# rogosprojects/klogs

Measured on AMD Instinct MI355X. Metric: filtered log GB/s (whole node) at 1/2/4/8 MI355X; % of HBM peak, higher is better.
Workload: dtype u8

## Files before the change

klogs_amd/csrc/klf_kernels.hip:

```cpp
#include <hip/hip_ext.h>
#include <hip/hip_runtime.h>

#include <cstdio>
#include <cstdlib>
#include <cstring>
#include <type_traits>

#include "klf_kernels.hpp"
#include "klf_ts.hpp"

namespace klf {
namespace {

#ifndef KLF_TIMELINE
#define KLF_TIMELINE 0
#endif
__device__ uint32_t g_abl_waves;
#if KLF_TIMELINE
__device__ uint64_t g_timeline[300000 * 8];
__device__ uint32_t g_lb_rounds, g_lb_spins;
#define KLF_STAMP(tile, k) do { if (threadIdx.x == 0 && (tile) < 300000) g_timeline[(size_t)(tile) * 8 + (k)] = __builtin_amdgcn_s_memtime(); } while (0)
#else
#define KLF_STAMP(tile, k) do { } while (0)
#endif
// ... 165 lines not shown
  }
  return x;
}

__device__ __forceinline__ uint32_t xad(uint32_t x, uint32_t c, uint32_t d) {
  uint32_t r;
  asm("v_xad_u32 %0, %1, %2, %3" : "=v"(r) : "v"(x), "s"(c), "v"(d));
  return r;
}
__device__ __forceinline__ uint32_t any_eq16(const uint4& v, uint32_t c4) {
  const uint32_t m = 0xFEFEFEFFu;
  return (xad(v.x, c4, m) | xad(v.y, c4, m) | xad(v.z, c4, m) | xad(v.w, c4, m)) & 0x80808080u;
}
__device__ __forceinline__ uint32_t eq_mask16(const uint4& v, uint32_t c4) {
  auto z = [c4](uint32_t x) {
    const uint32_t y = x ^ c4;
    const uint32_t f = ~(((y & 0x7F7F7F7Fu) + 0x7F7F7F7Fu) | y) & 0x80808080u;
    return (f * 0x00204081u) >> 28;
  };
  return z(v.x) | (z(v.y) << 4) | (z(v.z) << 8) | (z(v.w) << 12);
}

__device__ __forceinline__ uint32_t nor_and(uint32_t a, uint32_t b, uint32_t c) {
  uint32_t r;
  asm("v_bitop3_b32 %0, %1, %2, %3 bitop3:0x02" : "=v"(r) : "v"(a), "v"(b), "s"(c));
  return r;
}
__device__ __forceinline__ uint32_t eq_mask16_nl(const uint4& v) {
  auto z = [](uint32_t x) {
    const uint32_t t = xad(x & 0x7F7F7F7Fu, 0x0A0A0A0Au, 0x7F7F7F7Fu);
    const uint32_t f = nor_and(t, x, 0x80808080u);
    return (f * 0x00204081u) >> 28;
  };
  return z(v.x) | (z(v.y) << 4) | (z(v.z) << 8) | (z(v.w) << 12);
}

template <class T>
__device__ __forceinline__ T wave_max(T x) {
#pragma unroll
  for (int d = 32; d >= 1; d >>= 1) {
    const T o = __shfl_xor(x, d, 64);
    x = o > x ? o : x;
  }
  return x;
}

__device__ __forceinline__ void wave_lds_sync() { asm volatile("s_waitcnt lgkmcnt(0)" ::: "memory"); }

__global__ __launch_bounds__(256) void k_tiles(const SegDesc* segs, uint32_t nsegs, uint32_t ntiles,
                                               uint32_t* tile_seg) {
  for (uint32_t tile = blockIdx.x * 256 + threadIdx.x; tile < ntiles; tile += gridDim.x * 256)
    tile_seg[tile] = find_seg_by_tile(segs, nsegs, tile);
}

__device__ __forceinline__ uint32_t mul_hi_u24(uint32_t a, uint32_t b) {
  uint32_t r;
  asm("v_mul_hi_u32_u24 %0, %1, %2" : "=v"(r) : "s"(b), "v"(a));
  return r;
}
__device__ __forceinline__ uint32_t mul_u24(uint32_t a, uint32_t b) {
  uint32_t r;
  asm("v_mul_u32_u24 %0, %1, %2" : "=v"(r) : "s"(b), "v"(a));
  return r;
}
__device__ __forceinline__ uint32_t mad_u24(uint32_t a, uint32_t b, uint32_t c) {
  uint32_t r;
  asm("v_mad_u32_u24 %0, %1, %2, %3" : "=v"(r) : "v"(a), "s"(b), "v"(c));
  return r;
}
__device__ __forceinline__ uint32_t bfe_u32(uint32_t a, uint32_t off, uint32_t width) {
  uint32_t r;
  asm("v_bfe_u32 %0, %1, %2, %3" : "=v"(r) : "v"(a), "n"(off), "n"(width));
  return r;
}
__device__ __forceinline__ uint32_t shr_byte1(uint32_t w, uint32_t h) {
  uint32_t r;
  asm("v_lshrrev_b32_sdwa %0, %1, %2 dst_sel:DWORD dst_unused:UNUSED_PAD src0_sel:BYTE_1 src1_sel:DWORD"
      : "=v"(r) : "v"(h), "v"(w));
  return r;
}
#ifndef KLF_PARSE_UNALIGNED
#define KLF_PARSE_UNALIGNED 1
#endif
__device__ __forceinline__ bool parse_fast(const uint8_t* lds, uint32_t o, const uint32_t (&cut)[6], bool& since_ok) {
  uint32_t w[8];
  if (KLF_PARSE_UNALIGNED) {
    typedef uint32_t u32x4 __attribute__((ext_vector_type(4)));
    u32x4 x0, x1;
    __builtin_memcpy(&x0, lds + o, 16);
    __builtin_memcpy(&x1, lds + o + 16, 16);
    w[0] = x0.x; w[1] = x0.y; w[2] = x0.z; w[3] = x0.w;
    w[4] = x1.x; w[5] = x1.y; w[6] = x1.z; w[7] = x1.w;
  } else {
    const uint32_t* s32 = reinterpret_cast<const uint32_t*>(lds);
    const uint32_t base = o >> 2, sh = o & 3u;
    uint32_t prev = s32[base];
#pragma unroll
    for (int j = 0; j < 8; ++j) {
      const uint32_t nx = s32[base + j + 1];
      w[j] = __builtin_amdgcn_alignbyte(nx, prev, sh);
      prev = nx;
    }
  }
  const uint32_t sep = ((w[1] ^ 0x2D00002Du) & 0xFF0000FFu) | ((w[2] ^ 0x00540000u) & 0x00FF0000u) |
                       ((w[3] ^ 0x00003A00u) & 0x0000FF00u) | ((w[4] ^ 0x2E00003Au) & 0xFF0000FFu) |
                       ((w[7] ^ 0x00205A00u) & 0x00FFFF00u);
  const uint32_t p0 = __builtin_amdgcn_perm(0u, w[0], 0x00010203u);
  const uint32_t p1 = __builtin_amdgcn_perm(w[2], w[1], 0x01020405u);
  const uint32_t p2 = __builtin_amdgcn_perm(w[3], w[2], 0x03040607u);
  const uint32_t p3 = __builtin_amdgcn_perm(w[5], w[4], 0x01020405u);
  const uint32_t p4 = __builtin_amdgcn_perm(w[6], w[5], 0x02030405u);
  const uint32_t p5 = __builtin_amdgcn_perm(w[7], w[6], 0x02030C04u) | 0x00003000u;
  const uint32_t hi = ((p0 ^ 0x30303030u) | (p1 ^ 0x30303030u) | (p2 ^ 0x30303030u) | (p3 ^ 0x30303030u) |
                       (p4 ^ 0x30303030u) | (p5 ^ 0x30303030u)) & 0xF0F0F0F0u;
  const uint32_t lo = ((p0 + 0x06060606u) | (p1 + 0x06060606u) | (p2 + 0x06060606u) | (p3 + 0x06060606u) |
                       (p4 + 0x06060606u) | (p5 + 0x06060606u)) & 0x40404040u;
  if ((sep | hi | lo) != 0u) return false;
  if (p0 - 0x31393730u > 0x32303939u - 0x31393730u) return false;
  if ((p1 >> 16) - 0x3031u > 0x3132u - 0x3031u) return false;
  if ((p2 >> 16) > 0x3233u || (p2 & 0xFFFFu) > 0x3539u || (p3 >> 16) > 0x3539u) return false;
  if ((p1 & 0xFFFFu) - 0x3031u > 0x3238u - 0x3031u) {
    const uint32_t day = ((p1 >> 8) & 15u) * 10u + (p1 & 15u);
    const uint32_t month = ((p1 >> 24) & 15u) * 10u + ((p1 >> 16) & 15u);
    const uint32_t yy = ((p0 >> 8) & 15u) * 10u + (p0 & 15u);
    const uint32_t dim = month == 2u ? 28u + ((yy & 3u) == 0u ? 1u : 0u) : 30u + ((month + (month >> 3)) & 1u);
    if (day - 1u >= dim) return false;
  }
  const uint64_t a0 = (uint64_t)p0 << 32 | p1, a1 = (uint64_t)p2 << 32 | p3, a2 = (uint64_t)p4 << 32 | p5;
  const uint64_t c0 = (uint64_t)cut[0] << 32 | cut[1], c1 = (uint64_t)cut[2] << 32 | cut[3],
                 c2 = (uint64_t)cut[4] << 32 | cut[5];
  since_ok = a0 > c0 || (a0 == c0 && (a1 > c1 || (a1 == c1 && a2 >= c2)));
  return true;
}

#ifndef KLF_ABL
#define KLF_ABL 0
#endif
#ifndef KLF_SCAN_NT
#define KLF_SCAN_NT 1
#endif
#ifndef KLF_SCAN_PRIO
#define KLF_SCAN_PRIO 0
#endif
#ifndef KLF_NL_MASK
#define KLF_NL_MASK 1
#endif
#ifndef KLF_SCAN_BALLOT
#define KLF_SCAN_BALLOT 1
#endif
#ifndef KLF_SCAN_PACKSUM
#define KLF_SCAN_PACKSUM 1
#endif
#ifndef KLF_VERIFY_PAR
#define KLF_VERIFY_PAR 0
#endif
#ifndef KLF_HIT_INLINE
#define KLF_HIT_INLINE 0
#endif
#ifndef KLF_TS_INLINE
#define KLF_TS_INLINE 1
#endif
#ifndef KLF_SCAN_SUMSKIP
#define KLF_SCAN_SUMSKIP 1
#endif
typedef uint32_t klf_v4u __attribute__((ext_vector_type(4)));
__device__ __forceinline__ uint4 ld_nt(const uint4* p) {
  const klf_v4u v = __builtin_nontemporal_load(reinterpret_cast<const klf_v4u*>(p));
  return make_uint4(v.x, v.y, v.z, v.w);
}
#ifndef KLF_CG_NT
#define KLF_CG_NT 0
#endif
#ifndef KLF_CG_GRID
#define KLF_CG_GRID 8
#endif
#ifndef KLF_CG_PF2
#define KLF_CG_PF2 1
#endif
#ifndef KLF_COPY_U
#define KLF_COPY_U 1
#endif
#ifndef KLF_ANY_BATCH
#define KLF_ANY_BATCH 8
#endif
#ifndef KLF_SCAN_OCC
#define KLF_SCAN_OCC 3
#endif
constexpr int kScanPlain = 0, kScanLit = 1, kScanGen = 2;

__device__ __forceinline__ void copy_tile_runs(const uint8_t* s_buf, uint32_t* s_run, uint16_t* s_map, uint32_t nr,
                                               uint32_t kept, uint64_t obase, uint8_t* out, int lane);

template <int MODE, int QS, int QK, int QQ = 4, bool QA = false, bool FUSE = false>
__global__ __launch_bounds__(kThreads, MODE == kScanGen ? 3 : KLF_SCAN_OCC) void k_scan(RunArgs a, const uint32_t* __restrict__ tseg,
                                                               const SegDesc* __restrict__ segs) {
  static_assert(!FUSE || MODE == kScanPlain, "the fused compaction runs in the plain scan");
  constexpr bool LIT = MODE == kScanLit;
  constexpr bool GEN = MODE == kScanGen;
  constexpr bool ANC = GEN && QA;
  static_assert(QQ == 3 || QQ == 4, "3- or 4-byte grams");
  constexpr int kWaves = kThreads / 64;
  constexpr int kRows = kTile / 1024;
  constexpr int kPad = FUSE ? 16 : 0;
  __shared__ __attribute__((aligned(16))) uint8_t s_tile_all[kWaves][kPad + kTile + kHalo];
  __shared__ __attribute__((aligned(16))) uint32_t s_frun_all[FUSE ? kWaves : 1][FUSE ? kTcRuns : 1];
  __shared__ __attribute__((aligned(16))) uint16_t s_fmap_all[FUSE ? kWaves : 1][FUSE ? kTcChunks : 8];
  __shared__ __attribute__((aligned(16))) uint32_t s_list_all[kWaves][kSlotStride];
  __shared__ __attribute__((aligned(16))) uint32_t s_lit[kMaxFusedLiteral / 4 + 1];
  __shared__ uint4 s_gstat[GEN ? 1 : kWaves][kScanGroup];
  __shared__ uint32_t s_qf[GEN ? kQfWords : 1];
  __shared__ uint32_t s_h2[GEN ? kWaves : 1][1];
  const int t = threadIdx.x, lane = t & 63, wv = __builtin_amdgcn_readfirstlane(t >> 6);
  uint8_t* s_tile = s_tile_all[wv] + kPad;
  uint32_t* s_list = s_list_all[wv];
  uint32_t* err_flag = a.counters + 2;
  for (uint32_t i = t; i < kMaxFusedLiteral / 4 + 1; i += kThreads)
    s_lit[i] = (LIT && i < (a.lit_len + 3) / 4) ? a.lit_words[i] : 0u;
  if (GEN)
    for (uint32_t i = t; i < kQfWords; i += kThreads) s_qf[i] = a.pats.qf_bitmap[i];
  __syncthreads();
  const uint32_t nwaves = gridDim.x * kWaves;
  const bool abl = (KLF_ABL != 0) &&
                   __hip_atomic_load(&g_abl_waves, __ATOMIC_RELAXED, __HIP_MEMORY_SCOPE_AGENT) >= nwaves;
#define ABL(x) ((KLF_ABL & (x)) && abl)

  static_assert(kRows == 8, "KLF_ROWS lists the 8 prefetch rows");
#define KLF_ROWS(X) X(0) X(1) X(2) X(3) X(4) X(5) X(6) X(7)
#define KLF_DECL(r) uint4 pf##r;
  KLF_ROWS(KLF_DECL)
#undef KLF_DECL
#define KLF_LOAD(r) pf##r = (KLF_SCAN_NT && MODE != kScanPlain) ? ld_nt(&gp[r * 64 + lane]) : gp[r * 64 + lane];
#define KLF_STORE(r) l[r * 64 + lane] = pf##r;
  uint4 pfh = make_uint4(0, 0, 0, 0);
  auto next_tile = [&](uint32_t x) -> uint32_t {
    return (FUSE || (x % kScanGroup) != kScanGroup - 1) ? x + 1 : x + 1 + kScanGroup * (nwaves - 1);
  };
  const uint32_t gw = blockIdx.x * kWaves + wv;
  uint32_t tile = FUSE ? gw * a.fuse_range : gw * kScanGroup;
  const uint32_t tile_end = FUSE ? (tile + a.fuse_range < a.ntiles ? tile + a.fuse_range : a.ntiles) : a.ntiles;
  const uint32_t range_t0 = tile;
  uint4 stv = make_uint4(0, 0, 0, 0);
  uint32_t pf_s = 0;
  SegDesc pf_sd{};
  if (tile < a.ntiles) {
    pf_s = tseg[tile];
    pf_sd = segs[pf_s];
    const uint4* gp = reinterpret_cast<const uint4*>(a.bytes + pf_sd.base + (uint64_t)(tile - pf_sd.tile0) * kTile);
    KLF_ROWS(KLF_LOAD)
    if (lane < kHalo / 16) pfh = (KLF_SCAN_NT && MODE != kScanPlain) ? ld_nt(&gp[kTile / 16 + lane]) : gp[kTile / 16 + lane];
  }
  {
    const __amdgpu_buffer_rsrc_t none = __builtin_amdgcn_make_buffer_rsrc(a.slots, 0, 0, 0x00020000);
    __builtin_amdgcn_raw_buffer_store_b32(0u, none, 0x7FFF0000u, 0, 0);
  }
  bool any_defer = false;
  uint32_t wp_cur = 0, wp_end = 0;
  bool fz_known = false, fz_sel = false, fz_res_set = false;
  int32_t fz_crel = -1;
  uint64_t fz_obase = 0, fz_estart = 0, fz_res = 0, fz_part = 0, fz_rbase = 0;
  uint32_t fz_ext = 0;
  if (FUSE && tile < tile_end) {
    fz_rbase = pf_sd.base + (uint64_t)(tile - pf_sd.tile0) * kTile;
    fz_ext = a.fuse_ext0[gw];
  }
  auto fz_close = [&]() __attribute__((always_inline)) {
    if (!fz_res_set) {
      fz_res = fz_part;
      fz_res_set = true;
      fz_estart = fz_obase = fz_rbase + fz_part;
    }
    if (lane == 0) {
      a.fuse_ext[2 * (size_t)fz_ext] = fz_estart;
      a.fuse_ext[2 * (size_t)fz_ext + 1] = fz_obase - fz_estart;
    }
  };
  for (; tile < tile_end; tile = next_tile(tile)) {
    const uint32_t s = pf_s;
    const SegDesc sd = pf_sd;
    const int64_t rel_lo = (int64_t)(tile - sd.tile0) * kTile;
    const int64_t seg_len = (int64_t)sd.len;
    const int32_t tile_len = (int32_t)(seg_len - rel_lo < kTile ? seg_len - rel_lo : kTile);
    const bool first = rel_lo == 0;
    const bool last = rel_lo + kTile >= seg_len;
    const uint8_t* segp = a.bytes + sd.base;

    if (KLF_SCAN_PRIO) __builtin_amdgcn_s_setprio(KLF_SCAN_PRIO);
    {
      uint4* l = reinterpret_cast<uint4*>(s_tile);
      KLF_ROWS(KLF_STORE)
      if (lane < kHalo / 16) l[kTile / 16 + lane] = pfh;
      const uint32_t nx = next_tile(tile);
      if (nx < tile_end) {
        if (nx - sd.tile0 >= sd.ntiles) {
          pf_s = tseg[nx];
          pf_sd = segs[pf_s];
        }
        const uint4* gp = reinterpret_cast<const uint4*>(a.bytes + pf_sd.base + (uint64_t)(nx - pf_sd.tile0) * kTile);
        KLF_ROWS(KLF_LOAD)
        if (lane < kHalo / 16) pfh = (KLF_SCAN_NT && MODE != kScanPlain) ? ld_nt(&gp[kTile / 16 + lane]) : gp[kTile / 16 + lane];
      }
    }
    if (KLF_SCAN_PRIO) __builtin_amdgcn_s_setprio(0);
    wave_lds_sync();

    const uint32_t my0 = (uint32_t)lane * kLaneBytes;
    const int nvalid_s = tile_len - (int)my0;
    const int nvalid = nvalid_s <= 0 ? 0 : (nvalid_s >= kLaneBytes ? kLaneBytes : nvalid_s);
    const uint32_t pat = ANC ? a.pats.qf_anc_byte : a.lit_anchor_byte * 0x01010101u;
    const uint32_t afold = ANC ? a.pats.qf_anc_fold : 0u;
    auto or4 = [](const uint4& x, uint32_t f) { return make_uint4(x.x | f, x.y | f, x.z | f, x.w | f); };
    uint32_t nlc = 0, anc = 0;
    {
      const uint32_t rot = ((uint32_t)lane >> 1) & 7u;
#pragma unroll
      for (int v0 = 0; v0 < 8; v0 += KLF_ANY_BATCH) {
        uint4 xs[KLF_ANY_BATCH];
#pragma unroll
        for (int v = 0; v < KLF_ANY_BATCH; ++v)
          xs[v] = *reinterpret_cast<const uint4*>(s_tile + my0 + 16u * (((uint32_t)(v0 + v) + rot) & 7u));
#pragma unroll
        for (int v = 0; v < KLF_ANY_BATCH; ++v) {
          const uint32_t c = ((uint32_t)(v0 + v) + rot) & 7u;
          nlc |= any_eq16(xs[v], 0x0A0A0A0Au) ? (1u << c) : 0u;
          if (LIT && !ABL(2)) anc |= any_eq16(xs[v], pat) ? (1u << c) : 0u;
          if (ANC) anc |= any_eq16(afold ? or4(xs[v], afold) : xs[v], pat) ? (1u << c) : 0u;
        }
      }
      if (nvalid < kLaneBytes) {
        const uint32_t vm = (1u << ((nvalid + 15) >> 4)) - 1u;
        nlc &= vm;
        anc &= vm;
      }
    }
    if (ABL(64)) {
      asm volatile("" ::"v"(nlc | anc) : "memory");
      continue;
    }
    auto clip = [&](uint32_t e, uint32_t c) -> uint32_t {
      const int nv = nvalid - 16 * (int)c;
      return nv >= 16 ? e : (nv <= 0 ? 0u : (e & ((1u << nv) - 1u)));
    };
    uint32_t em[4] = {0u, 0u, 0u, 0u};
    for (uint32_t m = nlc; m; m &= m - 1u) {
      const uint32_t c = (uint32_t)__builtin_ctz(m);
      const uint4 x = *reinterpret_cast<const uint4*>(s_tile + my0 + 16u * c);
      const uint32_t e = clip(KLF_NL_MASK ? eq_mask16_nl(x) : eq_mask16(x, 0x0A0A0A0Au), c) << ((c & 1u) * 16u);
      const uint32_t q = c >> 1;
      em[0] |= q == 0 ? e : 0u;
      em[1] |= q == 1 ? e : 0u;
      em[2] |= q == 2 ? e : 0u;
      em[3] |= q == 3 ? e : 0u;
    }
    uint32_t st[4] = {em[0], em[1], em[2], em[3]};
    if (last && nvalid > 0 && (int)my0 + nvalid == tile_len) {
      const uint32_t eb = (uint32_t)nvalid - 1u, q = eb >> 5, bit = 1u << (eb & 31u);
      bool nl_at_end = false;
#pragma unroll
      for (int k = 0; k < 4; ++k)
        if ((uint32_t)k == q) {
          nl_at_end = (em[k] & bit) != 0u;
          em[k] |= bit;
          st[k] &= ~bit;
        }
      if (!abl) a.segout[s].frag = nl_at_end ? 0 : 1;
    }
    const uint32_t cnt = (uint32_t)(__popc(em[0]) + __popc(em[1]) + __popc(em[2]) + __popc(em[3]));
    const uint32_t incl = (KLF_SCAN_BALLOT && !__any(cnt > 1u))
                              ? cnt + __builtin_amdgcn_mbcnt_hi((uint32_t)(__ballot(cnt != 0u) >> 32),
                                                                __builtin_amdgcn_mbcnt_lo((uint32_t)__ballot(cnt != 0u), 0u))
                              : wave_incl_scan_add(cnt, lane);
    const uint32_t agg = (uint32_t)__builtin_amdgcn_readlane((int)incl, 63);
    const uint32_t k0 = first ? 0 : 1;
    const uint32_t k1 = last ? agg : agg + 1;
    const uint32_t nlines = k1 > k0 ? k1 - k0 : 0;
    const bool dense = nlines > (uint32_t)kSlots;
    uint32_t pool_base = 0;
    if (dense) {
      uint32_t pb = 0;
      if (lane == 0 && !abl) {
        pb = atomicAdd(&a.counters[kCtrPool], (nlines + 31u) & ~31u);
        if ((uint64_t)pb + nlines > a.pool_cap) atomicOr(err_flag, 1u);
      }
      pool_base = (uint32_t)__builtin_amdgcn_readlane((int)pb, 0);
    }
    const bool pool_ok = !dense || (uint64_t)pool_base + nlines <= a.pool_cap;
    uint32_t* const trec = a.slots + (size_t)tile * kRecStride;
    uint32_t* gslot = dense ? a.pool + pool_base : trec + kRecHead;

    uint32_t n_parsed = 0, n_since = 0, n_defer = 0, carry = 0, n_hit = 0;
    auto work = [&](uint32_t* list) __attribute__((always_inline)) {
      if (first && lane == 0) list[0] = 0u;
      {
        uint32_t kk = incl - cnt;
#pragma unroll
        for (int q = 0; q < 4; ++q) {
          for (uint32_t ev = em[q]; ev; ev &= ev - 1u) {
            const uint32_t b = (uint32_t)__builtin_ctz(ev);
            ++kk;
            if ((st[q] >> b) & 1u) list[kk - k0] = my0 + 32u * q + b + 1u;
          }
        }
      }
      if (dense) __threadfence_block();
      wave_lds_sync();
      for (uint32_t b0 = 0; b0 < nlines; b0 += 64) {
        const uint32_t j = b0 + (uint32_t)lane;
        if (j < nlines) {
          const uint32_t off = list[j];
          bool so = false, fast = false;
          if (ABL(1)) {
            fast = so = true;
          } else if (rel_lo + (int64_t)off + 31 <= seg_len) {
            fast = parse_fast(s_tile, off, a.since_dig, so);
          }
          if (FUSE && !fast) {
            TsResult tr;
            uint32_t plen = 0;
            const bool ok = parse_line_prefix(GlobalBytes{segp, rel_lo + (int64_t)off, seg_len}, tr, plen);
            const bool so2 = ok && !time_before(tr.sec, tr.nsec, a.since_sec, a.since_nsec);
            list[j] = off | ((uint32_t)make_meta(ok, so2, ok ? plen : 0u) << 16);
            if (ok && plen >= kPlenEscape) atomicOr(&a.counters[kCtrFuseBad], 1u);
            n_parsed += ok ? 1u : 0u;
            n_since += so2 ? 1u : 0u;
          } else {
            list[j] = fast ? (off | ((uint32_t)make_meta(true, so, 31) << 16)) : (off | kSlotDefer);
            n_parsed += fast ? 1u : 0u;
            n_since += (fast && so) ? 1u : 0u;
            n_defer += fast ? 0u : 1u;
          }
        }
      }
      if constexpr (MODE == kScanPlain && FUSE) {
        if (!dense) {
        wave_lds_sync();
        if (__any(n_defer != 0) && lane == 0) a.counters[kCtrFuseBad] = 1u;
        const uint64_t tin = sd.base + (uint64_t)rel_lo;
        if (first) {
          if (tile != range_t0) {
            fz_close();
            ++fz_ext;
          } else {
            fz_res_set = true;
          }
          fz_known = true;
          fz_sel = false;
          fz_crel = -1;
          fz_obase = fz_estart = tin;
          fz_part = 0;
        }
        const uint32_t span = nlines ? (list[0] & kSlotOff) : (uint32_t)tile_len;
        uint32_t clen = 0, csrc = 0;
        if (fz_known) {
          clen = f_carried(span, fz_sel, fz_crel);
          csrc = fz_crel > 0 ? (uint32_t)fz_crel : 0u;
        } else if (nlines) {
          fz_res = fz_part + span;
          fz_res_set = true;
          fz_obase = fz_estart = tin + span;
        }
        uint32_t* s_frun = s_frun_all[wv];
        uint32_t nr = 0, dacc = 0, lsel = 0;
        int32_t lcrel = -1;
        for (uint32_t b0 = 0; b0 < nlines; b0 += 64) {
          const uint32_t j = b0 + (uint32_t)lane;
          uint32_t src = 0, len = 0;
          if (j < nlines) {
            const uint32_t v = list[j], off = v & kSlotOff, mt = v >> 16;
            const bool sel = !(v & kSlotDefer) && (mt & Meta::kParsed) && (mt & Meta::kSince);
            const uint32_t c = off + (mt >> 2);
            const uint32_t e = j + 1 < nlines ? (list[j + 1] & kSlotOff) : (uint32_t)tile_len;
            if (sel && e > c) { src = c; len = e - c; }
            if (j + 1 == nlines) { lsel = sel ? 1u : 0u; lcrel = f_sat((int32_t)c - tile_len); }
          }
          const uint32_t incl = wave_incl_scan_add(len, lane);
          const uint64_t bm = __ballot(len != 0);
          const uint32_t idx = nr + (uint32_t)__popcll(bm & ((1ull << lane) - 1ull));
          if (len) s_frun[1 + idx] = src | ((clen + dacc + incl - len) << 16);
          nr += (uint32_t)__popcll(bm);
          dacc += (uint32_t)__builtin_amdgcn_readlane((int)incl, 63);
        }
        if (clen && lane == 0) s_frun[0] = csrc;
        const uint32_t kept = clen + dacc;
        if (kept) {
          if (fz_obase + kept + 16 > a.out_cap) {
            if (lane == 0) a.counters[kCtrFuseBad] = 1u;
          } else {
            copy_tile_runs(s_tile, clen ? s_frun : s_frun + 1, s_fmap_all[wv], nr + (clen ? 1u : 0u), kept, fz_obase,
                           a.out, lane);
// ... 52 lines not shown
            round(b0, w, o);
          }
          const uint32_t lastl = nlines ? ((nlines - 1u) & 63u) : 0u;
          const uint32_t psel = nlines ? (uint32_t)__builtin_amdgcn_readlane((int)lsel, (int)lastl) : 0u;
          const int32_t pcrel = nlines ? __builtin_amdgcn_readlane(lcrel, (int)lastl) : -1;
          const uint32_t span = nlines ? (list[0] & kSlotOff) : (uint32_t)tile_len;
          const uint32_t px = (dacc & 0x3FFFu) | ((span & 0x3FFFu) << 14) | ((nlines ? 1u : 0u) << 28) | (psel << 29);
          const uint32_t py = ((uint32_t)(uint16_t)(int16_t)pcrel) | (ns << 16);
          const uint32_t pz = (fits && nr + 1u <= (uint32_t)kRunSlots) ? nr : (uint32_t)kRunsRecompute;
          const __amdgpu_buffer_rsrc_t pr = __builtin_amdgcn_make_buffer_rsrc(a.trec + tile, 0, abl ? 0 : 16, 0x00020000);
          __builtin_amdgcn_raw_buffer_store_b128(u32x4p{px, py, pz, kPlanTag}, pr, lane ? 0x7FFF0000u : 0u, 0, 0);
        }
      }
      auto starts_upto = [&](int32_t pos) __attribute__((always_inline)) -> int {
        int lo = 0, hi = pos < 0 ? 0 : (int)nlines;
        while (lo < hi) {
          const int mid = (lo + hi) >> 1;
          if ((list[mid] & kSlotOff) <= (uint32_t)pos) lo = mid + 1; else hi = mid;
        }
        return lo;
      };
      auto attribute = [&](int32_t pos) __attribute__((always_inline)) {
        const int lo = starts_upto(pos);
        if (lo > 0) {
          const uint32_t v = list[lo - 1];
          const uint32_t mt = v >> 16;
          if (!(v & kSlotDefer) && (mt & Meta::kParsed) && (uint32_t)pos >= (v & kSlotOff) + (mt >> 2)) {
            atomicOr(&list[lo - 1], kSlotHit);
            ++n_hit;
          }
        } else {
          const uint32_t c1 = (uint32_t)(pos + 1 + (int32_t)kCarryBias);
          carry = carry > c1 ? carry : c1;
        }
      };
      if (LIT) {
        if (dense) __threadfence_block();
        wave_lds_sync();
        const uint32_t m = a.lit_len, ka = a.lit_anchor;
        auto check = [&](int32_t pos) __attribute__((always_inline)) {
          if (pos < 0 || pos >= tile_len || rel_lo + pos + (int64_t)m > seg_len) return;
          bool eq = true;
          if ((uint32_t)pos + m + 4 <= (uint32_t)(kTile + kHalo)) {
            const uint32_t* s32 = reinterpret_cast<const uint32_t*>(s_tile);
            const uint32_t sh = (uint32_t)pos & 3u;
            uint32_t wi = (uint32_t)pos >> 2;
            uint32_t prev = s32[wi];
            for (uint32_t k = 0; k < m && eq; k += 4) {
              const uint32_t nx = s32[++wi];
              const uint32_t got = __builtin_amdgcn_alignbyte(nx, prev, sh);
              prev = nx;
              const uint32_t nb = m - k < 4 ? m - k : 4;
              const uint32_t msk = nb == 4 ? 0xFFFFFFFFu : ((1u << (8 * nb)) - 1);
              eq = ((got ^ s_lit[k >> 2]) & msk) == 0;
            }
          } else {
            const uint8_t* lit = reinterpret_cast<const uint8_t*>(s_lit);
            for (uint32_t k = 0; k < m && eq; ++k) {
              const uint32_t o = (uint32_t)pos + k;
              const uint8_t c = o < (uint32_t)(kTile + kHalo) ? s_tile[o] : segp[rel_lo + o];
              eq = c == lit[k];
            }
          }
          if (!eq) return;
          attribute(pos);
        };
        for (uint32_t cm = anc; cm; cm &= cm - 1u) {
          const uint32_t c = (uint32_t)__builtin_ctz(cm);
          const uint4 x = *reinterpret_cast<const uint4*>(s_tile + my0 + 16u * c);
          for (uint32_t e = clip(eq_mask16(x, pat), c); e; e &= e - 1u)
            check((int32_t)(my0 + 16u * c + (uint32_t)__builtin_ctz(e)) - (int32_t)ka);
        }
        if (lane == 63 && ka > 0 && !last) {
          for (uint32_t jj = 0; jj < ka; ++jj) {
            const int64_t q = rel_lo + kTile + jj;
            if (q >= seg_len) break;
            const uint8_t c = jj < (uint32_t)kHalo ? s_tile[kTile + jj] : segp[q];
            if (c == a.lit_anchor_byte) check((int32_t)(kTile + jj) - (int32_t)ka);
          }
        }
        carry = wave_max(carry);
      }
      if (dense) __threadfence_block();
      wave_lds_sync();
    };
    if (ABL(128)) {
    } else if (!dense) {
      work(s_list);
    } else if (pool_ok && !abl) {
      if (FUSE && lane == 0) a.counters[kCtrFuseBad] = 1u;
      work(gslot);
    }

    uint32_t tile_hits = 0;
    bool hinl = false;
    uint32_t hit2 = 0;
    if (GEN) {
      const uint32_t fold = a.pats.qf_fold;
      const uint32_t* s32 = reinterpret_cast<const uint32_t*>(s_tile);
      struct Probe {
        uint32_t h, p, m, a;
      };
      constexpr bool kMidIdx = QQ == 3 && QK == 2;
      constexpr bool K3 = QK == 3 || QK == (int)kQfTwoLevel;
      constexpr bool TWO = QK == (int)kQfTwoLevel;
      static_assert(!TWO || QS == 4, "the two-level probe runs at stride 4");
      auto probe = [&](uint32_t g) __attribute__((always_inline)) -> Probe {
        const uint32_t gf = g | fold;
        const uint32_t f = K3 ? gf ^ bfe_u32(gf, 13, 11) : gf;
        Probe r;
        r.h = mul_u24(f, 0x9E3779u);
        if (QQ == 4) r.h = mad_u24(gf >> 8, 0x7F4A7Du, r.h);
        r.p = K3 ? mul_hi_u24(f, 0xC2B2AEu) : 0u;
        r.m = K3 ? mul_u24(f, 0x5BD1E9u) : 0u;
        r.a = TWO ? (((r.h >> 21) << 2) + kQfPairWords * 4u)
              : kMidIdx ? ((r.h >> 16) & ((kQfWords - 1u) << 2)) : ((r.h >> (32 - kQfBucketBits)) << 2);
        return r;
      };
      auto word = [&](const Probe& r) __attribute__((always_inline)) -> uint32_t {
        return *reinterpret_cast<const uint32_t*>(reinterpret_cast<const uint8_t*>(s_qf) + r.a);
      };
      auto test = [&](uint32_t w, const Probe& r) __attribute__((always_inline)) -> uint32_t {
        uint32_t t = K3 ? (w >> ((r.m >> 24) & 31u)) & (w >> (r.p & 31u))
                        : shr_byte1(w, r.h) & (w >> ((r.h >> 16) & 31u));
        if (K3) t &= w >> ((r.h >> 16) & 31u);
        if (TWO) t &= shr_byte1(w, r.m);
        return t;
      };
      auto hbits = [&](uint32_t g) __attribute__((always_inline)) -> uint32_t {
        const Probe r = probe(g);
        return test(word(r), r);
      };
      auto chunk_grams = [&](uint32_t c, auto&& f) __attribute__((always_inline)) {
        const uint32_t o0 = my0 + 16u * c;
        const uint4 x = *reinterpret_cast<const uint4*>(s_tile + o0);
        if constexpr (QS == 6) {
          f(x.x, 0);
          f(__builtin_amdgcn_alignbyte(x.z, x.y, 2u), 6);
          f(x.w, 12);
          return;
        }
        const uint32_t w4 = QS < 4 ? s32[(o0 >> 2) + 4] : 0u;
        const uint32_t w[5] = {x.x, x.y, x.z, x.w, w4};
#pragma unroll
        for (int d = 0; d < 4; ++d)
#pragma unroll
          for (int o = 0; o < 4; o += (QS < 4 ? QS : 4)) {
            if ((4 * d + o) % QS != 0) continue;
            f(o == 0 ? w[d] : __builtin_amdgcn_alignbyte(w[d + 1], w[d], o), 4 * d + o);
          }
      };
      uint32_t chit = 0;
      const uint32_t rot = ((uint32_t)lane >> 1) & 7u;
      uint32_t hq0 = 0, hq1 = 0, hq2 = 0, hq3 = 0;
      uint32_t xh = 0xFFFFFFFFu;
      if (TWO) {
        uint32_t sv = 0;
#pragma unroll
        for (int v = 0; v < (ABL(4) ? 0 : 8); v += 2) {
          const uint32_t ca = ((uint32_t)v + rot) & 7u, cb = ((uint32_t)v + 1u + rot) & 7u;
          const uint4 xa = *reinterpret_cast<const uint4*>(s_tile + my0 + 16u * ca);
          const uint4 xb = *reinterpret_cast<const uint4*>(s_tile + my0 + 16u * cb);
          const uint32_t g[8] = {xa.x, xa.y, xa.z, xa.w, xb.x, xb.y, xb.z, xb.w};
          uint32_t w[8];
#pragma unroll
          for (int k = 0; k < 8; ++k)
            w[k] = *reinterpret_cast<const uint32_t*>(reinterpret_cast<const uint8_t*>(s_qf) +
// ... 115 lines not shown
        const uint32_t tot = (uint32_t)__builtin_amdgcn_readlane((int)ih, 63);
        uint32_t ob = 0;
        if (tot > kHitSlots) {
          if (lane == 63) ob = atomicAdd(&a.counters[kCtrHits], tot - kHitSlots);
          ob = (uint32_t)__builtin_amdgcn_readlane((int)ob, 63);
        }
        uint16_t* hs = a.hslots + (size_t)tile * kHitSlots;
        hinl = KLF_HIT_INLINE && tot <= 2u && !dense && nlines != 1u;
        uint16_t* hd = hinl ? reinterpret_cast<uint16_t*>(s_h2[GEN ? wv : 0]) : hs;
        uint32_t k = ih - nh;
        if (xh != 0xFFFFFFFFu) {
          if (k < kHitSlots) {
            hd[k] = (uint16_t)xh;
          } else if ((uint64_t)ob + (k - kHitSlots) < a.qhits_cap) {
            a.qhits[ob + (k - kHitSlots)] = sd.base + (uint64_t)rel_lo + xh;
          } else {
            atomicOr(&a.counters[kCtrHitsOver], 1u);
          }
          ++k;
        }
        const uint32_t hq[4] = {hq0, hq1, hq2, hq3};
#pragma unroll
        for (int q = 0; q < 4; ++q)
          for (uint32_t m = hq[q]; m; m &= m - 1u, ++k) {
            const uint32_t off = my0 + 32u * q + (uint32_t)__builtin_ctz(m);
            if (k < kHitSlots) {
              hd[k] = (uint16_t)off;
            } else if ((uint64_t)ob + (k - kHitSlots) < a.qhits_cap) {
              a.qhits[ob + (k - kHitSlots)] = sd.base + (uint64_t)rel_lo + off;
            } else {
              atomicOr(&a.counters[kCtrHitsOver], 1u);
            }
          }
        tile_hits = tot < kHitSlots ? tot : kHitSlots;
        if (hinl) {
          wave_lds_sync();
          const uint32_t h2 = s_h2[GEN ? wv : 0][0];
          hit2 = tot > 1u ? h2 : (h2 & 0xFFFFu);
        }
      }
    }

#if KLF_SCAN_PACKSUM
    const uint32_t pq = (KLF_SCAN_BALLOT && nlines <= 64u)
                            ? (uint32_t)__popcll(__ballot(n_parsed != 0u)) | ((uint32_t)__popcll(__ballot(n_since != 0u)) << 16)
                            : wave_sum(n_parsed | (n_since << 16));
    const uint32_t pp = pq & 0xFFFFu, qq = pq >> 16;
    const uint32_t dd = __any(n_defer != 0) ? 1u : 0u;
#elif KLF_SCAN_SUMSKIP
    uint32_t pp = 0, qq = 0, dd = 0;
    if (nlines) { pp = wave_sum(n_parsed); qq = wave_sum(n_since); dd = wave_sum(n_defer); }
#else
    const uint32_t pp = wave_sum(n_parsed), qq = wave_sum(n_since), dd = wave_sum(n_defer);
#endif
    any_defer |= dd != 0;
    {
      const bool inl = KLF_TS_INLINE && !dense && nlines == 1u;
      const bool pooled = a.wave_pool && !dense && nlines >= 2u;
      const bool no_slots = (abl && !(KLF_ABL & (65536 | 131072))) || ABL(65536);
      uint32_t pb = dense ? pool_base : 0u, nunits = 0;
      uint32_t* sdst = trec;
      if (pooled && !no_slots) {
        const bool whole = nlines > 12u;
        const uint32_t need = whole ? (nlines + 31u) & ~31u : (nlines + 3u) & ~3u;
        if (whole) wp_cur = (wp_cur + 31u) & ~31u;
        if (wp_cur + need > wp_end) {
          const uint32_t ch = need > a.pool_chunk ? need : a.pool_chunk;
          uint32_t b = 0;
          if (lane == 0) b = atomicAdd(&a.counters[kCtrPool], ch);
          b = (uint32_t)__builtin_amdgcn_readfirstlane((int)b);
          wp_cur = b;
          wp_end = (uint64_t)b + ch <= a.pool_cap ? b + ch : b;
          if (wp_end == b && lane == 0) atomicOr(err_flag, 1u);
        }
        if (wp_cur + need <= wp_end) {
          pb = wp_cur;
          wp_cur += need;
          nunits = need / 4u;
          sdst = a.pool + pb;
        }
      } else if (!a.wave_pool && !no_slots && !dense && nlines > 1u - (KLF_TS_INLINE ? 0u : 1u)) {
        nunits = ((kRecHead + nlines + 31u) & ~31u) / 4u;
      }
      const uint32_t w0 = agg, w1 = (dense || pooled) ? pb : (inl ? s_list[0] : (hinl ? hit2 : 0u));
      const uint32_t w2 = (pp & 0xFFFFu) | (qq << 16);
      const bool hh = LIT && __any(n_hit != 0);
      const uint32_t w3 = (((dense || (pooled && nunits)) ? 1u : 0u) | (carry ? 2u : 0u) | (dd ? 4u : 0u) | (hh ? 8u : 0u) |
                           (inl ? kTsInline : 0u) | (hinl ? kTsHitInline : 0u)) |
                          ((uint32_t)(uint16_t)(GEN ? tile_hits : carry) << 16);
      const __amdgpu_buffer_rsrc_t rrs = __builtin_amdgcn_make_buffer_rsrc(sdst, 0, (int)(nunits * 16u), 0x00020000);
      typedef uint32_t u32x4v __attribute__((ext_vector_type(4)));
      const uint32_t ushift = a.wave_pool ? 0u : 1u;
      for (uint32_t u = (uint32_t)lane; u < (nunits > 64u ? 128u : 64u); u += 64) {
        const uint32_t us = u - ushift;
        const uint32_t li = u < ushift ? 0u : (4u * us < (uint32_t)kSlotStride - 4u ? 4u * us : (uint32_t)kSlotStride - 4u);
        const uint4 sl = *reinterpret_cast<const uint4*>(s_list + li);
        const u32x4v v = u >= ushift ? u32x4v{sl.x, sl.y, sl.z, sl.w} : u32x4v{w0, w1, w2, w3};
        __builtin_amdgcn_raw_buffer_store_b128(v, rrs, 16u * u, 0, 0);
      }
      const uint32_t gk = tile % kScanGroup, g0 = tile - gk;
      if (GEN) {
        if ((uint32_t)lane == gk) stv = make_uint4(w0, w1, w2, w3);
      } else {
        if (lane == 0) s_gstat[wv][gk] = make_uint4(w0, w1, w2, w3);
        wave_lds_sync();
      }
      const bool gend = gk == kScanGroup - 1 || tile + 1 >= a.ntiles;
      const uint32_t ng = a.ntiles - g0 < kScanGroup ? a.ntiles - g0 : kScanGroup;
      const __amdgpu_buffer_rsrc_t srs =
          __builtin_amdgcn_make_buffer_rsrc(a.tstat + g0, 0, (gend && (!abl || (KLF_ABL & 65536))) && !ABL(131072) ? (int)(16u * ng) : 0, 0x00020000);
      const uint4 gs = GEN ? stv : s_gstat[GEN ? 0 : wv][lane & (kScanGroup - 1)];
      __builtin_amdgcn_raw_buffer_store_b128(u32x4v{gs.x, gs.y, gs.z, gs.w}, srs, 16u * (uint32_t)lane, 0, 0);
    }
    asm volatile("" ::: "memory");
  }
  if (any_defer && lane == 0 && !abl) a.counters[kCtrDefer] = 1u;
  if (FUSE && range_t0 < tile_end) {
    fz_close();
    if (lane == 0) {
      uint64_t* ri = a.fuse_rinfo + 4 * (size_t)gw;
      ri[0] = fz_res;
      ri[1] = (fz_known ? 1u : 0u) | (fz_sel ? 2u : 0u);
      ri[2] = (uint64_t)(int64_t)fz_crel;
      ri[3] = fz_part;
    }
  }
  if (KLF_ABL != 0 && lane == 0) atomicAdd(&g_abl_waves, 1u);
#undef ABL
}

__device__ bool contains_bytes(const uint8_t* p, int64_t n, const uint8_t* lit, uint32_t m) {
  if ((int64_t)m > n) return false;
  for (int64_t i = 0; i + (int64_t)m <= n; ++i) {
    if (p[i] != lit[0]) continue;
    uint32_t k = 1;
    while (k < m && p[i + k] == lit[k]) ++k;
    if (k == m) return true;
  }
  return false;
}

__device__ bool ac_match(const DevPatterns& P, const uint8_t* p, int64_t n);
__device__ bool rx_match(const DevPatterns& P, uint32_t r, const uint8_t* p, int64_t n);
__device__ bool general_match(const DevPatterns& P, const uint8_t* p, int64_t n) {
  if (P.ac_states && ac_match(P, p, n)) return true;
  for (uint32_t r = 0; r < P.rx_count; ++r)
    if (rx_match(P, r, p, n)) return true;
  return false;
}

__device__ void count_pair(const RunArgs& a, uint64_t l, uint32_t s, uint32_t cid) {
  const uint64_t key = ((l << 20) | cid) + 1;
  const uint32_t mask = (1u << a.pairs_log2) - 1u;
  uint32_t h = (uint32_t)((key * 0x9E3779B97F4A7C15ull) >> 32) & mask;
  for (int probe = 0; probe < 128; ++probe) {
    const unsigned long long prev = atomicCAS(reinterpret_cast<unsigned long long*>(&a.pairs[h]), 0ull, key);
    if (prev == 0ull) {
      atomicAdd(&a.pcount[(size_t)s * a.pats.n_cids + cid], 1u);
      return;
    }
    if (prev == key) return;
    h = (h + 1u) & mask;
  }
  atomicAdd(&a.counters[kCtrPairsOver], 1u);
}

__device__ bool general_count(const RunArgs& a, const uint8_t* p, int64_t n, uint64_t l, uint32_t s) {
  const DevPatterns& P = a.pats;
  bool any = false;
  if (P.ac_states) {
    uint32_t st = 0;
    for (int64_t i = 0; i < n; ++i) {
      st = P.ac_next[(size_t)st * P.ac_classes + P.ac_class[p[i]]];
      if (!P.ac_accept[st]) continue;
      any = true;
      for (uint32_t t = P.ac_out[st] >= 0 ? st : P.ac_dict[st]; t; t = P.ac_dict[t]) count_pair(a, l, s, (uint32_t)P.ac_out[t]);
    }
  }
  for (uint32_t r = 0; r < P.rx_count; ++r)
    if (rx_match(P, r, p, n)) {
      any = true;
      count_pair(a, l, s, P.n_lits + r);
    }
  return any;
}

__device__ __forceinline__ uint32_t* slot_list(const RunArgs& a, const TileStat& ts, uint32_t tile) {
  return (ts.flags & 1u) ? a.pool + ts.pool_base
         : (ts.flags & kTsInline) ? reinterpret_cast<uint32_t*>(a.tstat + tile) + 1
         : a.slots ? a.slots + (size_t)tile * kRecStride + kRecHead : a.pool;
}
__device__ __forceinline__ uint32_t slot_at(const RunArgs& a, const TileStat& ts, uint32_t tile, uint32_t j) {
  return (ts.flags & kTsInline) ? ts.pool_base : slot_list(a, ts, tile)[j];
}

// ... 3054 lines not shown
```

Measured before the change: 5685.

## Defer timestamp parsing of sparse tiles to one batched pass per scan group

For tiles with at most four lines, each queue lane loads the candidate line's timestamp words into registers and postpones parsing until the end of the scan group. The whole group is then parsed at once across a quad of lanes per tile, and the slot results and per-tile stats are written directly to the pool/tstat. This is meant to cut the per-tile serial parse loop, its LDS sync and record store for sparse tiles. In exchange it adds eight live registers per lane, which may lower occupancy, plus more complex packing logic that must stay consistent with the existing record format.

```diff
diff --git a/klogs_amd/csrc/klf_kernels.hip b/klogs_amd/csrc/klf_kernels.hip
--- a/klogs_amd/csrc/klf_kernels.hip
+++ b/klogs_amd/csrc/klf_kernels.hip
@@ -271,8 +271,7 @@
 #ifndef KLF_PARSE_UNALIGNED
 #define KLF_PARSE_UNALIGNED 1
 #endif
-__device__ __forceinline__ bool parse_fast(const uint8_t* lds, uint32_t o, const uint32_t (&cut)[6], bool& since_ok) {
-  uint32_t w[8];
+__device__ __forceinline__ void parse_load(const uint8_t* lds, uint32_t o, uint32_t (&w)[8]) {
   if (KLF_PARSE_UNALIGNED) {
     typedef uint32_t u32x4 __attribute__((ext_vector_type(4)));
     u32x4 x0, x1;
@@ -291,6 +290,8 @@
       prev = nx;
     }
   }
+}
+__device__ __forceinline__ bool parse_words(const uint32_t (&w)[8], const uint32_t (&cut)[6], bool& since_ok) {
   const uint32_t sep = ((w[1] ^ 0x2D00002Du) & 0xFF0000FFu) | ((w[2] ^ 0x00540000u) & 0x00FF0000u) |
                        ((w[3] ^ 0x00003A00u) & 0x0000FF00u) | ((w[4] ^ 0x2E00003Au) & 0xFF0000FFu) |
                        ((w[7] ^ 0x00205A00u) & 0x00FFFF00u);
@@ -320,6 +321,11 @@
                  c2 = (uint64_t)cut[4] << 32 | cut[5];
   since_ok = a0 > c0 || (a0 == c0 && (a1 > c1 || (a1 == c1 && a2 >= c2)));
   return true;
+}
+__device__ __forceinline__ bool parse_fast(const uint8_t* lds, uint32_t o, const uint32_t (&cut)[6], bool& since_ok) {
+  uint32_t w[8];
+  parse_load(lds, o, w);
+  return parse_words(w, cut, since_ok);
 }
 
 #ifndef KLF_ABL
@@ -352,6 +358,12 @@
 #ifndef KLF_SCAN_SUMSKIP
 #define KLF_SCAN_SUMSKIP 1
 #endif
+#ifndef KLF_SCAN_TSGROUP
+#define KLF_SCAN_TSGROUP 1
+#endif
+constexpr uint32_t kTsQueue = 4;
+static_assert(kTsQueue == 4 && kTsQueue * kScanGroup <= 64, "a quad of queue lanes per tile of a group");
+constexpr uint32_t kTsqQueued = 1u << 17, kTsqValid = 1u << 16;
 typedef uint32_t klf_v4u __attribute__((ext_vector_type(4)));
 __device__ __forceinline__ uint4 ld_nt(const uint4* p) {
   const klf_v4u v = __builtin_nontemporal_load(reinterpret_cast<const klf_v4u*>(p));
@@ -428,7 +440,11 @@
   uint32_t tile = FUSE ? gw * a.fuse_range : gw * kScanGroup;
   const uint32_t tile_end = FUSE ? (tile + a.fuse_range < a.ntiles ? tile + a.fuse_range : a.ntiles) : a.ntiles;
   const uint32_t range_t0 = tile;
+  constexpr bool TSQ = GEN && !QA && QK != (int)kQfTwoLevel && KLF_SCAN_TSGROUP && KLF_TS_INLINE;
+  constexpr uint32_t kStLanes = TSQ ? kTsQueue : 1u;
   uint4 stv = make_uint4(0, 0, 0, 0);
+  uint32_t tq[8] = {0u, 0u, 0u, 0u, 0u, 0u, 0u, 0u};
+  uint32_t tqv = 0;
   uint32_t pf_s = 0;
   SegDesc pf_sd{};
   if (tile < a.ntiles) {
@@ -563,6 +579,9 @@
     const uint32_t k1 = last ? agg : agg + 1;
     const uint32_t nlines = k1 > k0 ? k1 - k0 : 0;
     const bool dense = nlines > (uint32_t)kSlots;
+    const uint32_t gk = tile % kScanGroup;
+    const bool tsq = TSQ && !abl && !dense && nlines >= 1u && nlines <= kTsQueue &&
+                     (nlines == 1u || (a.wave_pool && a.pool_cap <= 0x3FFFFFF0u));
     uint32_t pool_base = 0;
     if (dense) {
       uint32_t pb = 0;
@@ -592,7 +611,15 @@
       }
       if (dense) __threadfence_block();
       wave_lds_sync();
-      for (uint32_t b0 = 0; b0 < nlines; b0 += 64) {
+      if (tsq) {
+        const uint32_t j = (uint32_t)lane - kTsQueue * gk;
+        if (j < nlines) {
+          const uint32_t off = list[j];
+          parse_load(s_tile, off, tq);
+          tqv = off | kTsqQueued | (rel_lo + (int64_t)off + 31 <= seg_len ? kTsqValid : 0u);
+        }
+      }
+      for (uint32_t b0 = 0; b0 < (tsq ? 0u : nlines); b0 += 64) {
         const uint32_t j = b0 + (uint32_t)lane;
         if (j < nlines) {
           const uint32_t off = list[j];
@@ -811,7 +838,7 @@
         carry = wave_max(carry);
       }
       if (dense) __threadfence_block();
-      wave_lds_sync();
+      if (!tsq) wave_lds_sync();
     };
     if (ABL(128)) {
     } else if (!dense) {
@@ -1093,13 +1120,13 @@
       } else if (!a.wave_pool && !no_slots && !dense && nlines > 1u - (KLF_TS_INLINE ? 0u : 1u)) {
         nunits = ((kRecHead + nlines + 31u) & ~31u) / 4u;
       }
-      const uint32_t w0 = agg, w1 = (dense || pooled) ? pb : (inl ? s_list[0] : (hinl ? hit2 : 0u));
+      const uint32_t w0 = agg, w1 = (dense || pooled) ? pb : (inl ? (tsq ? 0u : s_list[0]) : (hinl ? hit2 : 0u));
       const uint32_t w2 = (pp & 0xFFFFu) | (qq << 16);
       const bool hh = LIT && __any(n_hit != 0);
       const uint32_t w3 = (((dense || (pooled && nunits)) ? 1u : 0u) | (carry ? 2u : 0u) | (dd ? 4u : 0u) | (hh ? 8u : 0u) |
                            (inl ? kTsInline : 0u) | (hinl ? kTsHitInline : 0u)) |
                           ((uint32_t)(uint16_t)(GEN ? tile_hits : carry) << 16);
-      const __amdgpu_buffer_rsrc_t rrs = __builtin_amdgcn_make_buffer_rsrc(sdst, 0, (int)(nunits * 16u), 0x00020000);
+      const __amdgpu_buffer_rsrc_t rrs = __builtin_amdgcn_make_buffer_rsrc(sdst, 0, tsq ? 0 : (int)(nunits * 16u), 0x00020000);
       typedef uint32_t u32x4v __attribute__((ext_vector_type(4)));
       const uint32_t ushift = a.wave_pool ? 0u : 1u;
       for (uint32_t u = (uint32_t)lane; u < (nunits > 64u ? 128u : 64u); u += 64) {
@@ -1109,9 +1136,9 @@
         const u32x4v v = u >= ushift ? u32x4v{sl.x, sl.y, sl.z, sl.w} : u32x4v{w0, w1, w2, w3};
         __builtin_amdgcn_raw_buffer_store_b128(v, rrs, 16u * u, 0, 0);
       }
-      const uint32_t gk = tile % kScanGroup, g0 = tile - gk;
+      const uint32_t g0 = tile - gk;
       if (GEN) {
-        if ((uint32_t)lane == gk) stv = make_uint4(w0, w1, w2, w3);
+        if ((uint32_t)lane == kStLanes * gk) stv = make_uint4(w0, w1, w2, w3);
       } else {
         if (lane == 0) s_gstat[wv][gk] = make_uint4(w0, w1, w2, w3);
         wave_lds_sync();
@@ -1120,8 +1147,38 @@
       const uint32_t ng = a.ntiles - g0 < kScanGroup ? a.ntiles - g0 : kScanGroup;
       const __amdgpu_buffer_rsrc_t srs =
           __builtin_amdgcn_make_buffer_rsrc(a.tstat + g0, 0, (gend && (!abl || (KLF_ABL & 65536))) && !ABL(131072) ? (int)(16u * ng) : 0, 0x00020000);
+      if constexpr (TSQ) {
+        uint32_t qslot = 0, qoff = 0xFFFFFFFFu;
+        if (gend && __any(tqv != 0u)) {
+          const bool qd = (tqv & kTsqQueued) != 0u;
+          uint32_t pk = 0;
+          if (qd) {
+            bool so = false;
+            const bool fast = (tqv & kTsqValid) && parse_words(tq, a.since_dig, so);
+            const uint32_t off = tqv & kSlotOff;
+            qslot = fast ? (off | ((uint32_t)make_meta(true, so, 31) << 16)) : (off | kSlotDefer);
+            pk = fast ? (1u | (so ? 0x10000u : 0u)) : 0x100u;
+          }
+          pk += dpp0<0xB1>(pk);
+          pk += dpp0<0x4E>(pk);
+          const uint32_t lw1 = dpp0<0x00>(stv.y), lw3 = dpp0<0x00>(stv.w);
+          if (qd && (lw3 & 1u)) qoff = 4u * (lw1 + ((uint32_t)lane & (kTsQueue - 1u)));
+          if (qd && ((uint32_t)lane & (kTsQueue - 1u)) == 0u) {
+            if (stv.w & kTsInline) stv.y = qslot;
+            stv.z = (pk & 0xFFu) | (pk & 0xFFFF0000u);
+            stv.w |= (pk & 0xFF00u) ? 4u : 0u;
+          }
+          any_defer |= __any((pk & 0xFF00u) != 0u);
+          tqv = 0;
+        }
+        const __amdgpu_buffer_rsrc_t prs =
+            __builtin_amdgcn_make_buffer_rsrc(a.pool, 0, gend ? (int)(uint32_t)(a.pool_cap * 4u) : 0, 0x00020000);
+        __builtin_amdgcn_raw_buffer_store_b32(qslot, prs, qoff, 0, 0);
+      }
       const uint4 gs = GEN ? stv : s_gstat[GEN ? 0 : wv][lane & (kScanGroup - 1)];
-      __builtin_amdgcn_raw_buffer_store_b128(u32x4v{gs.x, gs.y, gs.z, gs.w}, srs, 16u * (uint32_t)lane, 0, 0);
+      const uint32_t so16 = TSQ ? (((uint32_t)lane & (kTsQueue - 1u)) ? 0x7FFF0000u : 16u * ((uint32_t)lane / kTsQueue))
+                                : 16u * (uint32_t)lane;
+      __builtin_amdgcn_raw_buffer_store_b128(u32x4v{gs.x, gs.y, gs.z, gs.w}, srs, so16, 0, 0);
     }
     asm volatile("" ::: "memory");
   }
```

Measured after the change: 5571. 0.98x the previous value.
